# ericzzj1989/BALF

Hardware: NVIDIA B200
Metric: images/sec detect+NMS+top-k @640x480 (higher is better)
Workload: dtype fp16/tf32 operands (11-bit significand), fp32 accumulate

## Files before the change

### balf_b200/csrc/detector_tc.cuh

```cuda
#pragma once
#include <cuda_fp16.h>
#include "detector.cuh"
#include "umma.cuh"

namespace balf {
using namespace umma;

constexpr int kMerge32Ctas = 3;
constexpr int kRc16MinC = 32;
constexpr int TM = 128;
constexpr int NT2 = 256;
constexpr int kMaxSlot = 4;
constexpr int kMaxGemm = 6;

struct TcGemm {
    uint32_t goff;
    uint16_t nblk;
    uint16_t rows;
    uint16_t kb;
    uint16_t bias;
    uint16_t h16;
};
__host__ __device__ constexpr uint32_t tc_eb(int h16) { return h16 == 1 ? 2u : 4u; }
struct TcPlan {
// ... 180 lines not shown
            w_addr = r.wsm + slot * p.slot_bytes;
        }
        const uint64_t b_desc = desc_of(w_addr, b_lbo);
        fence_after_sync();
#pragma unroll
        for (int ks = 0; ks < KB / KSTEP; ++ks) {
            const uint32_t kchunk = (uint32_t)(b * KB) / EPC + (uint32_t)ks * 2u;
            const uint32_t a_off = ASW ? (kchunk / 8u) * (TM * 128u) + (kchunk % 8u) * 16u : kchunk * a_lbo;
            if (H16) mma_f16(d_tmem, a_desc + (a_off >> 4), b_desc + (((uint32_t)ks * 2u * b_lbo) >> 4), idesc, !(first && b == 0 && ks == 0));
            else mma_tf32(d_tmem, a_desc + (a_off >> 4), b_desc + (((uint32_t)ks * 2u * b_lbo) >> 4), idesc, !(first && b == 0 && ks == 0));
            if constexpr (X3) {
                mma_f16(d_tmem, a_desc + ((a_off + (uint32_t)(K / 8) * a_lbo) >> 4), b_desc + (((uint32_t)ks * 2u * b_lbo) >> 4), idesc, true);
                mma_f16(d_tmem, a_desc + (a_off >> 4), b_desc + ((((uint32_t)KB / 8u + (uint32_t)ks * 2u) * b_lbo) >> 4), idesc, true);
            }
        }
        if (BIAS && b + 1 == NBLK)
            mma_tf32(d_tmem, desc_of(ones_addr, TM * 16u), b_desc + ((((uint32_t)KB / EPC) * (X3 ? 2u : 1u) * b_lbo) >> 4), make_idesc_tf32(128, ROWS), true);
        if (!G::resident) { commit(&r.empty[slot]); ring_consumed<G::nslot>(r); }
    }
}

constexpr uint32_t kDescHiMn = ((uint32_t)(TM * 16u) >> 4) | (1u << 14);
__device__ __forceinline__ uint64_t desc_mn_of(uint32_t addr) {
    return ((uint64_t)kDescHiMn << 32) | (uint64_t)(((128u >> 4) << 16) | ((addr >> 4) & 0x3FFFu));
}
template <typename G, int GI, int C>
__device__ __forceinline__ void issue_mix_t(Ring& r, const TcPlan& p, uint32_t y_addr, uint32_t d_tmem) {
    uint32_t w_addr, slot = 0;
    if (G::resident) {
        w_addr = r.wsm + g_off<G>(GI);
    } else {
        ring_top_up<G::nslot>(r, p);
        slot = r.cslot;
        mbar_wait(&r.full[slot], r.cpar);
        w_addr = r.wsm + slot * p.slot_bytes;
    }
    fence_after_sync();
    constexpr uint32_t idesc = make_idesc_f16(64, C) | (1u << 16);
    constexpr uint32_t lo_off = (uint32_t)(C / 8) * TM * 16u;
    const uint64_t w_desc = desc_of(w_addr, 1024u);
    const uint64_t y_desc = desc_mn_of(y_addr);
#pragma unroll
    for (uint32_t u = 0; u < 2; ++u) {
#pragma unroll
        for (uint32_t ks = 0; ks < 4; ++ks) {
            const uint32_t yo = (32u * ks + 16u * u) * 16u;
            mma_f16(d_tmem + ((u * 16u) << 16), w_desc + ((ks * 2u * 1024u) >> 4), y_desc + (yo >> 4), idesc, ks > 0);
            if constexpr (G::x3) {
                mma_f16(d_tmem + ((u * 16u) << 16), w_desc + ((ks * 2u * 1024u) >> 4), y_desc + ((lo_off + yo) >> 4), idesc, true);
                mma_f16(d_tmem + ((u * 16u) << 16), w_desc + ((8192u + ks * 2u * 1024u) >> 4), y_desc + (yo >> 4), idesc, true);
            }
        }
    }
    if (!G::resident) { commit(&r.empty[slot]); ring_consumed<G::nslot>(r); }
}

__device__ __forceinline__ float ex2_approx(float x) {
    float y;
    asm("ex2.approx.ftz.f32 %0, %1;" : "=f"(y) : "f"(x));
    return y;
}
__device__ __forceinline__ unsigned long long pk2(float lo, float hi) {
    unsigned long long r;
    asm("mov.b64 %0, {%1, %2};" : "=l"(r) : "f"(lo), "f"(hi));
    return r;
}
__device__ __forceinline__ void upk2(unsigned long long r, float& lo, float& hi) { asm("mov.b64 {%0, %1}, %2;" : "=f"(lo), "=f"(hi) : "l"(r)); }
__device__ __forceinline__ unsigned long long fma2(unsigned long long a, unsigned long long b, unsigned long long c) {
    unsigned long long d;
    asm("fma.rn.f32x2 %0, %1, %2, %3;" : "=l"(d) : "l"(a), "l"(b), "l"(c));
    return d;
}
__device__ __forceinline__ unsigned long long add2(unsigned long long a, unsigned long long b) {
    unsigned long long d;
    asm("add.rn.f32x2 %0, %1, %2;" : "=l"(d) : "l"(a), "l"(b));
    return d;
}
__device__ __forceinline__ unsigned long long mul2(unsigned long long a, unsigned long long b) {
    unsigned long long d;
    asm("mul.rn.f32x2 %0, %1, %2;" : "=l"(d) : "l"(a), "l"(b));
    return d;
}
__device__ __forceinline__ void gelu_erf2(float& v0, float& v1) {
    const float t0 = fmaxf(-fabsf(v0), -5.6568542494923806f), t1 = fmaxf(-fabsf(v1), -5.6568542494923806f);
    const unsigned long long t = pk2(t0, t1);
    unsigned long long p = fma2(pk2(3.586947569e-04f, 3.586947569e-04f), t, pk2(6.316647399e-03f, 6.316647399e-03f));
    p = fma2(p, t, pk2(5.013782158e-02f, 5.013782158e-02f));
    p = fma2(p, t, pk2(-4.613807201e-01f, -4.613807201e-01f));
    p = fma2(p, t, pk2(1.150490999e+00f, 1.150490999e+00f));
    p = fma2(p, t, pk2(-1.0f, -1.0f));
    float p0, p1;
    upk2(p, p0, p1);
    const unsigned long long r = fma2(t, pk2(ex2_approx(p0), ex2_approx(p1)), pk2(fmaxf(v0, 0.0f), fmaxf(v1, 0.0f)));
    upk2(r, v0, v1);
}
template <int N, bool STATS>
__device__ __forceinline__ void gelu_row(float (&v)[N], float& sum, float& sq) {
    unsigned long long s2 = pk2(0.f, 0.f), q2 = pk2(0.f, 0.f);
#pragma unroll
    for (int i = 0; i < N; i += 2) {
        gelu_erf2(v[i], v[i + 1]);
        if (STATS) { const unsigned long long x = pk2(v[i], v[i + 1]); s2 = add2(s2, x); q2 = fma2(x, x, q2); }
    }
    if (STATS) { float a, b; upk2(s2, a, b); sum = a + b; upk2(q2, a, b); sq = a + b; }
}
template <int N>
__device__ __forceinline__ void norm_row(float (&v)[N], float rstd, float shift) {
    const unsigned long long r2 = pk2(rstd, rstd), h2 = pk2(shift, shift);
#pragma unroll
    for (int i = 0; i < N; i += 2) { const unsigned long long x = fma2(pk2(v[i], v[i + 1]), r2, h2); upk2(x, v[i], v[i + 1]); }
}
__device__ __forceinline__ float lrelu02(float v) { return v > 0.0f ? v : 0.2f * v; }

template <int CH>
__device__ __forceinline__ void ld_row(uint32_t taddr, float (&v)[CH]) {
    if constexpr (CH == 16) {
        tmem_ld16(taddr, v);
    } else {
#pragma unroll
        for (int c0 = 0; c0 < CH; c0 += 32) tmem_ld32(taddr + c0, *reinterpret_cast<float (*)[32]>(&v[c0]));
    }
    tmem_ld_wait();
}
template <int CH>
__device__ __forceinline__ void st_row(uint32_t taddr, const float (&v)[CH]) {
    if constexpr (CH == 16) {
        asm volatile(
            "tcgen05.st.sync.aligned.32x32b.x16.b32 [%0], {%1, %2, %3, %4, %5, %6, %7, %8, %9, %10, %11, %12, %13, %14, %15, %16};"
            :: "r"(taddr), "r"(__float_as_uint(v[0])), "r"(__float_as_uint(v[1])), "r"(__float_as_uint(v[2])), "r"(__float_as_uint(v[3])),
               "r"(__float_as_uint(v[4])), "r"(__float_as_uint(v[5])), "r"(__float_as_uint(v[6])), "r"(__float_as_uint(v[7])),
               "r"(__float_as_uint(v[8])), "r"(__float_as_uint(v[9])), "r"(__float_as_uint(v[10])), "r"(__float_as_uint(v[11])),
               "r"(__float_as_uint(v[12])), "r"(__float_as_uint(v[13])), "r"(__float_as_uint(v[14])), "r"(__float_as_uint(v[15]))
            : "memory");
    } else {
#pragma unroll
        for (int c0 = 0; c0 < CH; c0 += 32) tmem_st32(taddr + c0, *reinterpret_cast<const float (*)[32]>(&v[c0]));
    }
    tmem_st_wait();
}

template <int CH>
__device__ __forceinline__ void row_to_a(const float (&v)[CH], float* region, int row, int col0) {
#pragma unroll
    for (int j = 0; j < CH / 4; ++j)
        *reinterpret_cast<float4*>(region + ((size_t)(col0 / 4 + j) * TM + row) * 4) =
            to_tf32(make_float4(v[4 * j], v[4 * j + 1], v[4 * j + 2], v[4 * j + 3]));
}

__device__ __forceinline__ void split_h2(float a, float b, uint32_t& hi, uint32_t& lo) {
    asm("cvt.rn.satfinite.f16x2.f32 %0, %1, %2;" : "=r"(hi) : "f"(b), "f"(a));
    const float2 f = __half22float2(*reinterpret_cast<const __half2*>(&hi));
    asm("cvt.rn.satfinite.f16x2.f32 %0, %1, %2;" : "=r"(lo) : "f"(b - f.y), "f"(a - f.x));
}
template <int CH, int LOC = 0>
__device__ __forceinline__ void row_to_a16(const float (&v)[CH], float* region, int row, int col0) {
#pragma unroll
    for (int j = 0; j < CH / 8; ++j) {
        uint32_t h[4], l[4];
#pragma unroll
        for (int e = 0; e < 4; ++e) {
            if constexpr (LOC > 0) split_h2(v[8 * j + 2 * e], v[8 * j + 2 * e + 1], h[e], l[e]);
            else asm("cvt.rn.satfinite.f16x2.f32 %0, %1, %2;" : "=r"(h[e]) : "f"(v[8 * j + 2 * e + 1]), "f"(v[8 * j + 2 * e]));
        }
        *reinterpret_cast<uint4*>(region + ((size_t)(col0 / 8 + j) * TM + row) * 4) = make_uint4(h[0], h[1], h[2], h[3]);
        if constexpr (LOC > 0) *reinterpret_cast<uint4*>(region + ((size_t)(LOC + col0 / 8 + j) * TM + row) * 4) = make_uint4(l[0], l[1], l[2], l[3]);
    }
}
// ... 338 lines not shown
        }
        pf.v[0] = make_float4(v[0], v[1], v[2], v[3]);
    } else {
        constexpr int N = InputPf<CIN, TPR>::N;
        const float4* src = reinterpret_cast<const float4*>(xin + (img * npix + pix) * CIN) + half * N;
        if constexpr (PAIR) {
            pair_load<N>(src, valid, pf.v);
        } else {
#pragma unroll
            for (int j = 0; j < N; ++j) pf.v[j] = valid ? __ldg(src + j) : make_float4(0.f, 0.f, 0.f, 0.f);
        }
    }
}
template <int CIN, bool PAIR = true, int TPR = 2, int H16 = 0>
__device__ __forceinline__ void store_input_row(const InputPf<CIN, TPR>& pf, float* dst, int row, int half) {
    if constexpr (H16 == 3 && CIN >= 8) {
        constexpr int N16 = CIN / (8 * TPR);
#pragma unroll
        for (int j = 0; j < N16; ++j) *reinterpret_cast<float4*>(dst + ((size_t)(half * N16 + j) * TM + row) * 4) = pf.v[j];
        return;
    }
    if constexpr (CIN < 8) {
        if (half < 2) *reinterpret_cast<float4*>(dst + ((size_t)half * TM + row) * 4) = to_tf32(pf.v[0]);
    } else {
        constexpr int N = InputPf<CIN, TPR>::N;
#pragma unroll
        for (int j = 0; j < N; j += 2) {
            float4 c0 = pf.v[j], c1 = pf.v[j + 1];
            if constexpr (PAIR) pair_unswap(c0, c1);
            if constexpr (H16 != 0) {
                const float e[8] = {c0.x, c0.y, c0.z, c0.w, c1.x, c1.y, c1.z, c1.w};
                uint32_t h[4], l[4];
#pragma unroll
                for (int q = 0; q < 4; ++q) {
                    if constexpr (H16 == 2) split_h2(e[2 * q], e[2 * q + 1], h[q], l[q]);
                    else asm("cvt.rn.satfinite.f16x2.f32 %0, %1, %2;" : "=r"(h[q]) : "f"(e[2 * q + 1]), "f"(e[2 * q]));
                }
                *reinterpret_cast<uint4*>(dst + ((size_t)((half * N + j) / 2) * TM + row) * 4) = make_uint4(h[0], h[1], h[2], h[3]);
                if constexpr (H16 == 2)
                    *reinterpret_cast<uint4*>(dst + ((size_t)(CIN / 8 + (half * N + j) / 2) * TM + row) * 4) = make_uint4(l[0], l[1], l[2], l[3]);
            } else {
                *reinterpret_cast<float4*>(dst + ((size_t)(half * N + j) * TM + row) * 4) = to_tf32(c0);
                *reinterpret_cast<float4*>(dst + ((size_t)(half * N + j + 1) * TM + row) * 4) = to_tf32(c1);
            }
        }
    }
}


constexpr int kConv0Off = 64;
template <int CIN, int C>
__device__ __forceinline__ void conv0_stage_weights(const DownW& w, float* vec) {
    for (int i = threadIdx.x; i < CIN * C; i += NT2) vec[kConv0Off + i] = __ldg(w.conv0_w + i);
    for (int i = threadIdx.x; i < C; i += NT2) vec[kConv0Off + CIN * C + i] = __ldg(w.conv0_b + i);
}
template <int CIN, int C, int CH>
__device__ __forceinline__ void conv0_row(const float4 x, const float* vec, int col0, float (&v)[CH]) {
    const float xs[4] = {x.x, x.y, x.z, x.w};
    const float* cw = vec + kConv0Off + col0;
#pragma unroll
    for (int i = 0; i < CH; i += 4) {
        const float4 b = *reinterpret_cast<const float4*>(cw + CIN * C + i);
        unsigned long long a01 = pk2(b.x, b.y), a23 = pk2(b.z, b.w);
#pragma unroll
        for (int k = 0; k < CIN; ++k) {
            const float4 wv = *reinterpret_cast<const float4*>(cw + k * C + i);
            const unsigned long long xk = pk2(xs[k], xs[k]);
            a01 = fma2(pk2(wv.x, wv.y), xk, a01);
            a23 = fma2(pk2(wv.z, wv.w), xk, a23);
        }
        upk2(a01, v[i], v[i + 1]);
        upk2(a23, v[i + 2], v[i + 3]);
#pragma unroll
        for (int j = 0; j < 4; ++j) v[i + j] = fmaxf(v[i + j], 0.f);
    }
}

template <int C, int PX> struct BranchCfg {
    static constexpr int TPR = C == 32 ? 1 : C == 256 ? 4 : 2;
    static constexpr int groups = C == 32 ? 5 : C == 64 ? 2 : 1;
    static constexpr int NTG = TM * TPR;
    static constexpr int CH = C / TPR;
    static constexpr uint32_t region = (uint32_t)TM * C * (PX ? 4u : 2u);
    static constexpr bool park_u = C <= 128;
    static constexpr bool h16_out = C <= 128;
    static constexpr int col_u = 0;
    static constexpr int col_y = park_u ? C : 0;
    static constexpr int ncols = groups * tc_cols(col_y + 2 * C) > 512 ? col_y + 2 * C : tc_cols(col_y + 2 * C);
    static constexpr uint32_t xch = TPR == 1 ? 0u : 2u * TPR * TM * 8u;
    static constexpr int SC = TPR == 1 ? 16 : TPR == 4 ? (CH < 32 ? CH : 32) : (CH > 64 ? 64 : CH);
};

template <int CIN, int C, int BR, int PX>
__device__ __forceinline__ void tc_branch_body(const float* __restrict__ xin, const DownW& w, const TcPlan& plan, const UnitGeom& geo,
                                               float* __restrict__ out, float* __restrict__ scratch, unsigned char* smem) {
    using Cfg = BranchCfg<C, PX>;
    using G = BranchG<CIN, C, PX>;
    constexpr int CH = Cfg::CH, NG = Cfg::groups, TPR = Cfg::TPR, NTG = Cfg::NTG, SC = Cfg::SC;
    constexpr bool X3 = PX != 0;
    constexpr int LOC = X3 ? C / 8 : 0;
    constexpr bool XH = !X3 && CIN >= 8;
    constexpr bool CL16 = !Cfg::h16_out && !X3;
    float* const rt = CL16 ? scratch : out;
    constexpr int XM = XH ? 3 : X3 ? 2 : 1;
    static_assert(NG == 1 || G::resident, "tile groups share resident weights (no ring state per group)");
    static_assert(CH % SC == 0 && SC % 16 == 0, "sub-chunking");
    TcShared s = carve(smem, Cfg::region, plan, NG, Cfg::xch);
    const int grp = NG == 1 ? 0 : (int)(threadIdx.x / NTG);
    const int tid = threadIdx.x - grp * NTG, row = tid & (TM - 1), half = tid >> 7;
    const int vblock = (int)blockIdx.x * NG + grp, vgrid = (int)gridDim.x * NG;
    const int ntiles = (geo.total_units + 1) / 2;
    const uint32_t my_tiles = vblock < ntiles ? (ntiles - 1 - vblock) / vgrid + 1 : 0;
    const DownW::Branch& br = w.br[BR];
    if (grp == 0) {
        for (int i = tid; i < C; i += NTG) { s.vec[i] = __ldg(br.gn_w + i); s.vec[256 + i] = __ldg(br.gn_b + i); }
        for (int i = tid; i < 64; i += NTG) s.vec[512 + i] = __ldg(br.gd_b + i) + 1.0f;
        if constexpr (CIN < 8) {
            for (int i = tid; i < CIN * C; i += NTG) s.vec[kConv0Off + i] = __ldg(w.conv0_w + i);
            for (int i = tid; i < C; i += NTG) s.vec[kConv0Off + CIN * C + i] = __ldg(w.conv0_b + i);
        }
    }
    Ring ring;
    const bool w0 = __shfl_sync(0xffffffffu, tid >> 5, 0) == 0;
    tc_prologue<G::nslot>(s, tc_cols(Cfg::ncols * NG), ring, plan, my_tiles, w0 && grp == 0);
    if (NG > 1) {
        if (grp > 0 && w0 && elect_one()) mbar_wait(&s.full[0], 0);
        s.region += (size_t)grp * (Cfg::region / 4);
        s.xch += (size_t)grp * (Cfg::xch / 8);
        if (grp > 0) s.done = &s.gdone[grp];
    }
    const uint32_t tm = *s.tmem_slot + (uint32_t)(grp * Cfg::ncols);
    const uint32_t lane_base = tm + ((uint32_t)(row & ~31) << 16);
    const uint32_t region_addr = smem_u32(s.region), ones_addr = smem_u32(s.ones);
    const int ug = (row & 31) >> 4, tok = (row >> 5) * 16 + (row & 15);
    const int col0 = half * CH;
    const float* const mix_b1p = s.vec + 512 + tok;
    const int ostride = (BR == 0 ? geo.fw : 1) * C;
    const size_t npix = (size_t)geo.h * geo.w;
    uint32_t phase = 0, xb = 0;
    int it = 0;
    InputPf<CIN, TPR> pf;
    auto coords = [&](int tt, bool& vld, int& im, int& px) {
        const int un = 2 * tt + ug;
        vld = un < geo.total_units;
        im = vld ? fast_div(un, geo.upi, geo.inv_upi) : 0;
        px = unit_pixel<BR>(geo, vld ? un - im * geo.upi : 0, tok);
    };
    auto stats_of = [&](const float (&v)[CH], float& sum, float& sq) {
        unsigned long long s2 = pk2(0.f, 0.f), q2 = pk2(0.f, 0.f);
#pragma unroll
        for (int i = 0; i < CH; i += 2) {
            const unsigned long long x = pk2(v[i], v[i + 1]);
            s2 = add2(s2, x); q2 = fma2(x, x, q2);
        }
        float a, b;
        upk2(s2, a, b); sum = a + b;
        upk2(q2, a, b); sq = a + b;
    };
    bool nvld = false; int nim = 0, npx = 0;
    if (InputPf<CIN, TPR>::enabled && vblock < ntiles) {
        coords(vblock, nvld, nim, npx);
        fetch_input_row<CIN, true, TPR, XH>(xin, npix, (size_t)nim, npx, nvld, half, pf);
    }
    for (int t = vblock; t < ntiles; t += vgrid, ++it) {
        TC_TRACE(plan, it, 0);
        bool valid; int img, pix;
        if (InputPf<CIN, TPR>::enabled && (TPR > 1 || !X3)) { valid = nvld; img = nim; pix = npx; }
        else coords(t, valid, img, pix);
        float* orow = rt + ((size_t)img * npix + pix) * C + col0;
        float v[CH], rstd, shift;
        if constexpr (CIN < 8) {
            const float4 xv = pf.v[0];
            if (t + vgrid < ntiles) {
                coords(t + vgrid, nvld, nim, npx);
                fetch_input_row<CIN, true, TPR, XH>(xin, npix, (size_t)nim, npx, nvld, half, pf);
            }
            conv0_row<CIN, C, CH>(xv, s.vec, col0, v);
        } else {
            if (InputPf<CIN, TPR>::enabled) {
                store_input_row<CIN, true, TPR, XM>(pf, s.region, row, half);
                if (t + vgrid < ntiles) {
                    coords(t + vgrid, nvld, nim, npx);
                    fetch_input_row<CIN, true, TPR, XH>(xin, npix, (size_t)nim, npx, nvld, half, pf);
                }
            } else {
                load_input_row<CIN, TPR, XM>(xin, npix, (size_t)img, pix, valid, s.region, row, half);
            }
            TC_TRACE(plan, it, 1);
            sync_for_mma<NG, NTG>(grp);
            if (w0 && elect_one()) { issue_linear_t<G, BG_CONV0>(ring, plan, region_addr, ones_addr, tm + Cfg::col_y, true); commit(s.done); }
            TC_TRACE(plan, it, 2);
            wait_done_ring<G, NG, NTG>(s.done, phase, ring, plan, w0, grp);
            TC_TRACE(plan, it, 3);
            ld_row<CH>(lane_base + Cfg::col_y + col0, v);
#pragma unroll
            for (int i = 0; i < CH; ++i) v[i] = fmaxf(v[i], 0.f);
        }
        {
            float sum, sq;
            stats_of(v, sum, sq);
            row_stats<NG, TPR>(sum, sq, s.xch + (xb++ & 1) * TPR * TM, row, half, C, rstd, shift, grp);
            norm_row<CH>(v, rstd, shift);
            row_to_a16<CH, LOC>(v, s.region, row, col0);
        }
        TC_TRACE(plan, it, 4);
        sync_for_mma<NG, NTG>(grp);
        if (w0 && elect_one()) { issue_linear_t<G, BG_PD1>(ring, plan, region_addr, ones_addr, tm + Cfg::col_u, true); commit(s.done); }
        TC_TRACE(plan, it, 5);
        wait_done_ring<G, NG, NTG>(s.done, phase, ring, plan, w0, grp);
        TC_TRACE(plan, it, 6);
        {
            ld_row<CH>(lane_base + Cfg::col_u + col0, v);
            float sum = 0.f, sq = 0.f;
            gelu_row<CH, true>(v, sum, sq);
            if (Cfg::park_u) st_row<CH>(lane_base + Cfg::col_u + col0, v);
            else if constexpr (CH % 32 == 0 && !X3) oct_store<CH / 4>(rt, ((size_t)img * npix + pix) * C + col0, ostride, v, valid);
            else pair_store<CH / 4>(rt, ((size_t)img * npix + pix) * C + col0, v, valid);
            row_stats<NG, TPR>(sum, sq, s.xch + (xb++ & 1) * TPR * TM, row, half, C, rstd, shift, grp);
            norm_row<CH>(v, rstd, shift);
            row_to_a16<CH, LOC>(v, s.region, row, col0);
        }
        TC_TRACE(plan, it, 7);
        sync_for_mma<NG, NTG>(grp);
        if (w0 && elect_one()) {
            issue_linear_t<G, BG_D1A>(ring, plan, region_addr, ones_addr, tm + Cfg::col_y, true);
            issue_linear_t<G, BG_D1B>(ring, plan, region_addr, ones_addr, tm + Cfg::col_y + C, true);
            commit(s.done);
        }
        TC_TRACE(plan, it, 8);
        wait_done_ring<G, NG, NTG>(s.done, phase, ring, plan, w0, grp);
        TC_TRACE(plan, it, 9);
        {
            ld_row<CH>(lane_base + Cfg::col_y + col0, v);
            { float d0, d1; gelu_row<CH, false>(v, d0, d1); }
            st_row<CH>(lane_base + Cfg::col_y + col0, v);
            ld_row<CH>(lane_base + Cfg::col_y + C + col0, v);
            float sum = 0.f, sq = 0.f;
            gelu_row<CH, true>(v, sum, sq);
            row_stats<NG, TPR>(sum, sq, s.xch + (xb++ & 1) * TPR * TM, row, half, C, rstd, shift, grp);
            norm_row<CH>(v, rstd, shift);
#pragma unroll
            for (int i = 0; i < CH; i += 4) {
                const float4 gw = *reinterpret_cast<const float4*>(s.vec + col0 + i), gb = *reinterpret_cast<const float4*>(s.vec + 256 + col0 + i);
                upk2(fma2(pk2(v[i], v[i + 1]), pk2(gw.x, gw.y), pk2(gb.x, gb.y)), v[i], v[i + 1]);
                upk2(fma2(pk2(v[i + 2], v[i + 3]), pk2(gw.z, gw.w), pk2(gb.z, gb.w)), v[i + 2], v[i + 3]);
            }
            row_to_a16<CH, LOC>(v, s.region, row, col0);
        }
        TC_TRACE(plan, it, 10);
        sync_for_mma<NG, NTG>(grp);
        if (w0 && elect_one()) { issue_mix_t<G, BG_WM, C>(ring, plan, region_addr, tm + Cfg::col_y + C); commit(s.done); }
        TC_TRACE(plan, it, 11);
        wait_done_ring<G, NG, NTG>(s.done, phase, ring, plan, w0, grp);
        TC_TRACE(plan, it, 12);
        {
#pragma unroll 1
            for (int c = 0; c < CH; c += SC) {
                float y1[SC], y2[SC];
                ld_row<SC>(lane_base + Cfg::col_y + col0 + c, y1);
                ld_row<SC>(lane_base + Cfg::col_y + C + col0 + c, y2);
                const float mix_b1 = *mix_b1p;
                const unsigned long long b2 = pk2(mix_b1, mix_b1);
#pragma unroll
                for (int i = 0; i < SC; i += 2) upk2(mul2(pk2(y1[i], y1[i + 1]), add2(pk2(y2[i], y2[i + 1]), b2)), y2[i], y2[i + 1]);
                row_to_a16<SC, LOC>(y2, s.region, row, col0 + c);
            }
        }
        TC_TRACE(plan, it, 13);
        sync_for_mma<NG, NTG>(grp);
        if (w0 && elect_one()) { issue_linear_t<G, BG_D2>(ring, plan, region_addr, ones_addr, tm + Cfg::col_y, true); commit(s.done); }
        TC_TRACE(plan, it, 14);
        wait_done_ring<G, NG, NTG>(s.done, phase, ring, plan, w0, grp);
        TC_TRACE(plan, it, 15);
        {
            const bool odd = (threadIdx.x & 1) != 0;
            const size_t own_base = Cfg::h16_out ? ((size_t)img * npix + (pix & ~(TM - 1))) * C * (X3 ? 2 : 1)
                                                 : ((size_t)img * npix + pix) * C;
            const size_t oth_base = __shfl_xor_sync(0xffffffffu, (unsigned long long)own_base, 1);
            const size_t base_a = odd ? oth_base : own_base, base_b = odd ? own_base : oth_base;
            if constexpr (CL16 && CH % 64 == 0) {
                float hv[CH / 2];
#pragma unroll
                for (int c = 0; c < CH; c += SC) {
                    float a[SC];
                    ld_row<SC>(lane_base + Cfg::col_y + col0 + c, a);
#pragma unroll
                    for (int j0 = 0; j0 < SC / 4; j0 += 8) {
                        float4 t8[8];
                        pair_load<8>(reinterpret_cast<const float4*>(orow + c) + j0, valid, t8);
#pragma unroll
                        for (int j = 0; j < 8; j += 2) {
                            pair_unswap(t8[j], t8[j + 1]);
#pragma unroll
                            for (int u2 = 0; u2 < 2; ++u2) {
                                const float4 rr = t8[j + u2];
                                const int i = 4 * (j0 + j + u2);
                                uint32_t h0, h1;
                                asm("cvt.rn.satfinite.f16x2.f32 %0, %1, %2;" : "=r"(h0) : "f"(a[i + 1] + rr.y), "f"(a[i] + rr.x));
                                asm("cvt.rn.satfinite.f16x2.f32 %0, %1, %2;" : "=r"(h1) : "f"(a[i + 3] + rr.w), "f"(a[i + 2] + rr.z));
                                hv[(c + i) / 2] = __uint_as_float(h0);
                                hv[(c + i) / 2 + 1] = __uint_as_float(h1);
                            }
                        }
                    }
                }
                oct_store<CH / 8>(out, (((size_t)img * npix + pix) * C + col0) / 2, ostride / 2, hv, valid);
            } else
#pragma unroll 1
            for (int c = 0; c < CH; c += SC) {
                float a[SC], r[SC];
                ld_row<SC>(lane_base + Cfg::col_y + col0 + c, a);
                if (Cfg::park_u) ld_row<SC>(lane_base + Cfg::col_u + col0 + c, r);
                if constexpr (Cfg::h16_out) {
                    __half* tile = reinterpret_cast<__half*>(out) + own_base + (size_t)(pix & (TM - 1)) * 8;
#pragma unroll
                    for (int j = 0; j < SC / 8; ++j) {
                        uint32_t h[4], l[4];
#pragma unroll
                        for (int e = 0; e < 4; ++e) {
                            float lo, hi;
                            upk2(add2(pk2(a[8 * j + 2 * e], a[8 * j + 2 * e + 1]), pk2(r[8 * j + 2 * e], r[8 * j + 2 * e + 1])), lo, hi);
                            if constexpr (X3) split_h2(lo, hi, h[e], l[e]);
                            else asm("cvt.rn.satfinite.f16x2.f32 %0, %1, %2;" : "=r"(h[e]) : "f"(hi), "f"(lo));
                        }
                        if (valid) {
                            *reinterpret_cast<uint4*>(tile + (size_t)((col0 + c) / 8 + j) * (TM * 8)) = make_uint4(h[0], h[1], h[2], h[3]);
                            if constexpr (X3)
                                *reinterpret_cast<uint4*>(tile + (size_t)(C / 8 + (col0 + c) / 8 + j) * (TM * 8)) = make_uint4(l[0], l[1], l[2], l[3]);
                        }
                    }
                    continue;
                }
                float4 o[SC / 4];
                if constexpr (!Cfg::park_u) {
                    float4* rq = reinterpret_cast<float4*>(r);
#pragma unroll
                    for (int j0 = 0; j0 < SC / 4; j0 += 8) {
                        float4 t8[8];
                        pair_load<8>(reinterpret_cast<const float4*>(orow + c) + j0, valid, t8);
#pragma unroll
                        for (int j = 0; j < 8; j += 2) { pair_unswap(t8[j], t8[j + 1]); rq[j0 + j] = t8[j]; rq[j0 + j + 1] = t8[j + 1]; }
                    }
                }
#pragma unroll
                for (int j = 0; j < SC / 4; ++j) {
                    float4 res;
                    res = make_float4(r[4 * j], r[4 * j + 1], r[4 * j + 2], r[4 * j + 3]);
                    o[j] = make_float4(a[4 * j] + res.x, a[4 * j + 1] + res.y, a[4 * j + 2] + res.z, a[4 * j + 3] + res.w);
                    if (BR == 1 && !X3) o[j] = to_tf32_clean(o[j]);
                }
                if constexpr (SC % 32 == 0 && !X3) {
                    oct_store<SC / 4>(out, ((size_t)img * npix + pix) * C + col0 + c, ostride, reinterpret_cast<const float*>(o), valid);
                    continue;
                }
// ... 805 lines not shown
    if (g.bias)
        tc_pack_bias_kernel<<<cdiv(g.rows, 128), 128, 0, st>>>(wT, ld, n0, g.rows, k_real, bias, f.beta, f.alpha, f.add,
                                                               blob + g.goff + (size_t)g.rows * k_pad / (g.h16 == 1 ? 2 : 1));
    else if (p.ebias_off && bias) {
        const int slot = gi == MG_CONV0 ? 0 : gi == MG_PD2B ? 1 : gi == MG_RC1 ? 2 : 3;
        tc_pack_bias_kernel<<<cdiv(g.rows, 128), 128, 0, st>>>(wT, ld, n0, g.rows, k_real, bias, f.beta, f.alpha, f.add,
                                                               blob + p.ebias_off + (size_t)slot * g.rows * 4);
    }
}

int tc_pack_weights(const balf_detector_arch& a, const DetW& w, float* blob, cudaStream_t st) {
    BALF_CUDA_OK(cudaMemsetAsync(blob, 0, tc_blob_floats(a) * sizeof(float), st));
    const Fold none{nullptr, nullptr, nullptr, nullptr};
    for (int px = 0; px < 2; ++px) {
    TcPlans P;
    tc_build_plans(a, blob, &P, px);
    for (int l = 0; l < 4; ++l) {
        const int ci = a.dims[l], c = a.dims[l + 1];
        const DownW& d = w.down[l];
        for (int b = 0; b < 2; ++b) {
            const TcPlan& p = P.branch[l][b];
            const DownW::Branch& r = d.br[b];
            tc_pack_one(p, BG_CONV0, d.conv0_w, c, 0, ci, d.conv0_b, none, blob, st);
            tc_pack_one(p, BG_PD1, d.pd1_w, 2 * c, b * c, c, d.pd1_b, Fold{d.pn_w, d.pn_b, nullptr, nullptr}, blob, st);
            tc_pack_one(p, BG_D1A, r.d1_w, 2 * c, 0, c, r.d1_b, Fold{r.n_w, r.n_b, nullptr, nullptr}, blob, st);
            tc_pack_one(p, BG_D1B, r.d1_w, 2 * c, c, c, r.d1_b, Fold{r.n_w, r.n_b, nullptr, nullptr}, blob, st);
            tc_pack_one(p, BG_WM, r.gd_w, 64, 0, 64, nullptr, none, blob, st);
            tc_pack_one(p, BG_D2, r.d2_w, c, 0, c, r.d2_b, none, blob, st);
        }
        const TcPlan& m = P.merge[l];
        tc_pack_one(m, MG_CONV0, d.conv0_w, c, 0, ci, d.conv0_b, none, blob, st);
        tc_pack_one(m, MG_PD2A, d.pd2_w, c, 0, c, nullptr, none, blob, st);
        tc_pack_one(m, MG_PD2B, d.pd2_w + (size_t)c * c, c, 0, c, d.pd2_b, none, blob, st);
        tc_pack_one(m, MG_RC1, d.rc1_w, c, 0, c, d.rc1_b, Fold{d.rn_w, d.rn_b, nullptr, nullptr}, blob, st);
        tc_pack_one(m, MG_RC2, d.rc2_w, c, 0, c, d.rc2_b, none, blob, st);
    }
    tc_pack_one(P.head, HG_C2, w.down[3].c2_w, a.dims[4], 0, a.dims[4], w.down[3].c2_b, none, blob, st);
    tc_pack_one(P.head, HG_DENSE, w.head.w, kHeadPad, 0, a.dims[4], w.head.b, Fold{nullptr, nullptr, w.head.alpha, w.head.beta}, blob, st);
    }
    BALF_LAUNCH_OK();
    return 0;
}

#endif

static int g_num_sms = 0;
static int num_sms() {
    if (!g_num_sms) {
        int dev = 0;
        cudaGetDevice(&dev);
        cudaDeviceGetAttribute(&g_num_sms, cudaDevAttrMultiProcessorCount, dev);
        if (g_num_sms <= 0) g_num_sms = 148;
    }
    return g_num_sms;
}

template <typename K>
static int tc_launch_cfg(K kernel, size_t smem, int tmem_cols, int ntiles, int* grid, int groups = 1, int group_threads = NT2) {
    BALF_REQUIRE(smem <= 227 * 1024, "internal: tc kernel needs %zu bytes of shared memory", smem);
    BALF_CUDA_OK(cudaFuncSetAttribute(kernel, cudaFuncAttributeMaxDynamicSharedMemorySize, (int)smem));
    BALF_CUDA_OK(cudaFuncSetAttribute(kernel, cudaFuncAttributePreferredSharedMemoryCarveout, cudaSharedmemCarveoutMaxShared));
    cudaFuncAttributes fa;
    BALF_CUDA_OK(cudaFuncGetAttributes(&fa, kernel));
    const int regs_per_cta = ((fa.numRegs + 7) / 8 * 8) * group_threads * groups;
    ntiles = (ntiles + groups - 1) / groups;
    int per_sm = (int)((227 * 1024) / (smem + 1024));
    if (regs_per_cta > 0 && 65536 / regs_per_cta < per_sm) per_sm = 65536 / regs_per_cta;
    if (512 / tmem_cols < per_sm) per_sm = 512 / tmem_cols;
    if (per_sm < 1) per_sm = 1;
    const int cap = num_sms() * per_sm;
    *grid = ntiles < cap ? ntiles : cap;
    return 0;
}


template <int CIN, int C, int PX>
static int tc_launch_branches(const float* xin, const DownW& w, const TcPlans& P, int level, const UnitGeom& g, int ntiles,
                              float* u, float* v, float* su, float* sv, cudaStream_t st) {
    using Cfg = BranchCfg<C, PX>;
    constexpr int NG = Cfg::groups;
    int grid = 0;
    for (int b = 0; b < 2; ++b) {
        const TcPlan& p = P.branch[level][b];
        const size_t smem = tc_smem_bytes(Cfg::region, p, NG, Cfg::xch);
        if (b == 0) {
            if (int e = tc_launch_cfg(tc_branch_kernel<CIN, C, 0, PX>, smem, tc_cols(Cfg::ncols * NG), ntiles, &grid, NG, Cfg::NTG)) return e;
            ProfScope ps(C == 32 ? "det_branch_grid_c32" : C == 64 ? "det_branch_grid_c64" : C == 128 ? "det_branch_grid_c128" : "det_branch_grid_c256", st);
            tc_branch_kernel<CIN, C, 0, PX><<<grid, Cfg::NTG * NG, smem, st>>>(xin, w, p, g, u, su);
        } else {
            if (int e = tc_launch_cfg(tc_branch_kernel<CIN, C, 1, PX>, smem, tc_cols(Cfg::ncols * NG), ntiles, &grid, NG, Cfg::NTG)) return e;
            ProfScope ps(C == 32 ? "det_branch_block_c32" : C == 64 ? "det_branch_block_c64" : C == 128 ? "det_branch_block_c128" : "det_branch_block_c256", st);
            tc_branch_kernel<CIN, C, 1, PX><<<grid, Cfg::NTG * NG, smem, st>>>(xin, w, p, g, v, sv);
        }
    }
    return 0;
}

template <int CIN, int C, int PX>
static int tc_run_level(const float* xin, const DownW& w, const TcPlans& P, int level, int Bc, int h, int wd,
                        float* u, float* v, float* r, float* q, float* partial, cudaStream_t st, int r16) {
    UnitGeom g{h, wd, h / 8, wd / 8, h * wd / 64, Bc * (h * wd / 64), 1.0f / (float)(h * wd / 64), 1.0f / (float)(wd / 8), 1.0f / (float)(wd / 8)};
    BALF_REQUIRE(g.total_units < (1 << 23), "internal: %d units in one pass exceed the fast_div range", g.total_units);
    const int ntiles = (g.total_units + 1) / 2;
    int grid = 0;
    BALF_REQUIRE((plan_matches<BranchG<CIN, C, PX>>(P.branch[level][0]) && plan_matches<BranchG<CIN, C, PX>>(P.branch[level][1]) &&
                  plan_matches<MergeG<CIN, C, PX>>(P.merge[level])), "internal: compile-time and packed GEMM plans differ (level %d)", level);
    if (int e = tc_launch_branches<CIN, C, PX>(xin, w, P, level, g, ntiles, u, v, r, q, st)) return e;
    if constexpr (C <= 64) {
        const TcPlan& p = P.merge[level];
        BALF_REQUIRE(g.total_units % 2 == 0, "internal: odd unit count at stage %d", level);
        const size_t smem = tc_smem_bytes(MergeBulkCfg<CIN, C, PX>::region, p, 1, MergeBulkCfg<CIN, C, PX>::xch);
        if (int e = tc_launch_cfg(tc_merge_bulk_kernel<CIN, C, PX>, smem, MergeBulkCfg<CIN, C, PX>::ncols, ntiles, &grid)) return e;
        ProfScope ps(C == 32 ? "det_merge_c32" : "det_merge_c64", st);
        tc_merge_bulk_kernel<CIN, C, PX><<<grid, NT2, smem, st>>>(xin, w, p, g, u, v, r, q, partial);
    } else {
        const TcPlan& p = P.merge[level];
        BALF_REQUIRE((!MergeCfg<C, PX>::bulk_uv || g.total_units % 2 == 0), "internal: odd unit count at stage %d", level);
        const size_t smem = tc_smem_bytes(MergeCfg<C, PX>::region, p, 1, MergeCfg<C, PX>::xch);
        if (int e = tc_launch_cfg(tc_merge_kernel<CIN, C, PX>, smem, MergeCfg<C, PX>::ncols, ntiles, &grid, 1, MergeCfg<C, PX>::NT)) return e;
        ProfScope ps(C == 128 ? "det_merge_c128" : "det_merge_c256", st);
        tc_merge_kernel<CIN, C, PX><<<grid, MergeCfg<C, PX>::NT, smem, st>>>(xin, p, g, u, v, r, q, partial, r16);
    }
    BALF_COUNT_LAUNCH(3);
    BALF_LAUNCH_OK();
    return 0;
}

template <int PX>
int tc_level_px(int level, const float* xin, const DownW& w, const balf_detector_arch& a, const float* blob,
                int Bc, int h, int wd, float* u, float* v, float* r, float* q, float* partial, cudaStream_t st, int r16) {
    TcPlans P;
    tc_build_plans(a, blob, &P, PX);
    switch (level) {
        case 0: return tc_run_level<3, 32, PX>(xin, w, P, 0, Bc, h, wd, u, v, r, q, partial, st, r16);
        case 1: return tc_run_level<32, 64, PX>(xin, w, P, 1, Bc, h, wd, u, v, r, q, partial, st, r16);
        case 2: return tc_run_level<64, 128, PX>(xin, w, P, 2, Bc, h, wd, u, v, r, q, partial, st, r16);
        default: return tc_run_level<128, 256, PX>(xin, w, P, 3, Bc, h, wd, u, v, r, q, partial, st, r16);
    }
}
template <int PX>
int tc_head_px(const float* r, const float* q, const float* scale, const balf_detector_arch& a,
               const float* blob, int Bc, int hc, int wc, float* logits, float* prob, cudaStream_t st, int r16) {
    TcPlans P;
    tc_build_plans(a, blob, &P, PX);
    UnitGeom g{hc, wc, hc / 8, wc / 8, hc * wc / 64, Bc * (hc * wc / 64), 1.0f / (float)(hc * wc / 64), 1.0f / (float)(wc / 8), 1.0f / (float)(wc / 8)};
    BALF_REQUIRE(g.total_units < (1 << 23), "internal: %d units in one pass exceed the fast_div range", g.total_units);
    const int ntiles = (g.total_units + 1) / 2;
    const size_t smem = tc_smem_bytes((uint32_t)TM * 256 * 4, P.head);
    int grid = 0;
    BALF_REQUIRE((plan_matches<HeadG<256, PX>>(P.head)), "internal: compile-time and packed GEMM plans differ (head)");
    if (int e = tc_launch_cfg(tc_head_kernel<256, PX>, smem, 512, ntiles, &grid)) return e;
    {
        ProfScope ps("det_head", st);
        tc_head_kernel<256, PX><<<grid, NT2, smem, st>>>(r, q, scale, P.head, g, a.cell, logits, prob, PX ? 0 : r16);
    }
    BALF_COUNT_LAUNCH(1);
    BALF_LAUNCH_OK();
    return 0;
}

#ifdef BALF_TC_MAIN
extern template int tc_level_px<1>(int, const float*, const DownW&, const balf_detector_arch&, const float*, int, int, int, float*, float*,
                                   float*, float*, float*, cudaStream_t, int);
extern template int tc_head_px<1>(const float*, const float*, const float*, const balf_detector_arch&, const float*, int, int, int, float*,
                                  float*, cudaStream_t, int);

int tc_run_level_dispatch(int level, const float* xin, const DownW& w, const balf_detector_arch& a, const float* blob,
// ... 21 lines not shown
```

Baseline: 5238.

## Double-buffer C32 operand region and overlap next tile's conv0 with MMAs

For the C=32 branch (where conv.0 runs on CUDA cores), the shared operand region is doubled so the next tile's conv0, row-norm and fp16 staging run while the final linear MMA of the current tile is in flight. The GELU pass over the first TMEM half moves after the mix MMA issue so it overlaps that MMA. The erf clamp in gelu_erf2 is removed to save an instruction per pair. Costs are more shared memory per CTA, which can reduce occupancy, and possible range issues in the polynomial for large |x| without the clamp.

Result: faster. 5388, median of 6 (+2.9%).

```diff
diff --git a/balf_b200/csrc/detector_tc.cuh b/balf_b200/csrc/detector_tc.cuh
--- a/balf_b200/csrc/detector_tc.cuh
+++ b/balf_b200/csrc/detector_tc.cuh
@@ -286,7 +286,7 @@
     return d;
 }
 __device__ __forceinline__ void gelu_erf2(float& v0, float& v1) {
-    const float t0 = fmaxf(-fabsf(v0), -5.6568542494923806f), t1 = fmaxf(-fabsf(v1), -5.6568542494923806f);
+    const float t0 = -fabsf(v0), t1 = -fabsf(v1);
     const unsigned long long t = pk2(t0, t1);
     unsigned long long p = fma2(pk2(3.586947569e-04f, 3.586947569e-04f), t, pk2(6.316647399e-03f, 6.316647399e-03f));
     p = fma2(p, t, pk2(5.013782158e-02f, 5.013782158e-02f));
@@ -791,6 +791,7 @@
     static constexpr int NTG = TM * TPR;
     static constexpr int CH = C / TPR;
     static constexpr uint32_t region = (uint32_t)TM * C * (PX ? 4u : 2u);
+    static constexpr int nbuf = C == 32 ? 2 : 1;
     static constexpr bool park_u = C <= 128;
     static constexpr bool h16_out = C <= 128;
     static constexpr int col_u = 0;
@@ -814,7 +815,8 @@
     constexpr int XM = XH ? 3 : X3 ? 2 : 1;
     static_assert(NG == 1 || G::resident, "tile groups share resident weights (no ring state per group)");
     static_assert(CH % SC == 0 && SC % 16 == 0, "sub-chunking");
-    TcShared s = carve(smem, Cfg::region, plan, NG, Cfg::xch);
+    static_assert((Cfg::nbuf == 2) == (CIN < 8), "two operand regions exactly where conv.0 runs on the CUDA cores");
+    TcShared s = carve(smem, Cfg::nbuf * Cfg::region, plan, NG, Cfg::xch);
     const int grp = NG == 1 ? 0 : (int)(threadIdx.x / NTG);
     const int tid = threadIdx.x - grp * NTG, row = tid & (TM - 1), half = tid >> 7;
     const int vblock = (int)blockIdx.x * NG + grp, vgrid = (int)gridDim.x * NG;
@@ -834,13 +836,13 @@
     tc_prologue<G::nslot>(s, tc_cols(Cfg::ncols * NG), ring, plan, my_tiles, w0 && grp == 0);
     if (NG > 1) {
         if (grp > 0 && w0 && elect_one()) mbar_wait(&s.full[0], 0);
-        s.region += (size_t)grp * (Cfg::region / 4);
+        s.region += (size_t)grp * (Cfg::nbuf * Cfg::region / 4);
         s.xch += (size_t)grp * (Cfg::xch / 8);
         if (grp > 0) s.done = &s.gdone[grp];
     }
     const uint32_t tm = *s.tmem_slot + (uint32_t)(grp * Cfg::ncols);
     const uint32_t lane_base = tm + ((uint32_t)(row & ~31) << 16);
-    const uint32_t region_addr = smem_u32(s.region), ones_addr = smem_u32(s.ones);
+    const uint32_t region0_addr = smem_u32(s.region), ones_addr = smem_u32(s.ones);
     const int ug = (row & 31) >> 4, tok = (row >> 5) * 16 + (row & 15);
     const int col0 = half * CH;
     const float* const mix_b1p = s.vec + 512 + tok;
@@ -871,29 +873,49 @@
         coords(vblock, nvld, nim, npx);
         fetch_input_row<CIN, true, TPR, XH>(xin, npix, (size_t)nim, npx, nvld, half, pf);
     }
+    bool cvld = false; int cim = 0, cpx = 0;
+    auto stage1_input = [&](int tn, float* dst) {
+        if constexpr (CIN < 8) {
+            const float4 xv = pf.v[0];
+            cvld = nvld; cim = nim; cpx = npx;
+            if (tn + vgrid < ntiles) {
+                coords(tn + vgrid, nvld, nim, npx);
+                fetch_input_row<CIN, true, TPR, XH>(xin, npix, (size_t)nim, npx, nvld, half, pf);
+            }
+            float v[CH], rstd, shift, sum, sq;
+            conv0_row<CIN, C, CH>(xv, s.vec, col0, v);
+            stats_of(v, sum, sq);
+            row_stats<NG, TPR>(sum, sq, s.xch + (xb++ & 1) * TPR * TM, row, half, C, rstd, shift, grp);
+            norm_row<CH>(v, rstd, shift);
+            row_to_a16<CH, LOC>(v, dst, row, col0);
+        }
+    };
+    if constexpr (CIN < 8) {
+        if (vblock < ntiles) stage1_input(vblock, s.region);
+    }
     for (int t = vblock; t < ntiles; t += vgrid, ++it) {
         TC_TRACE(plan, it, 0);
+        const uint32_t rb = (uint32_t)(it & (Cfg::nbuf - 1));
+        float* const region = s.region + (size_t)rb * (Cfg::region / 4);
+        const uint32_t region_addr = region0_addr + rb * Cfg::region;
         bool valid; int img, pix;
-        if (InputPf<CIN, TPR>::enabled && (TPR > 1 || !X3)) { valid = nvld; img = nim; pix = npx; }
-        else coords(t, valid, img, pix);
+        if (InputPf<CIN, TPR>::enabled && (TPR > 1 || !X3)) {
+            if constexpr (CIN < 8) { valid = cvld; img = cim; pix = cpx; }
+            else { valid = nvld; img = nim; pix = npx; }
+        } else {
+            coords(t, valid, img, pix);
+        }
         float* orow = rt + ((size_t)img * npix + pix) * C + col0;
         float v[CH], rstd, shift;
-        if constexpr (CIN < 8) {
-            const float4 xv = pf.v[0];
-            if (t + vgrid < ntiles) {
-                coords(t + vgrid, nvld, nim, npx);
-                fetch_input_row<CIN, true, TPR, XH>(xin, npix, (size_t)nim, npx, nvld, half, pf);
-            }
-            conv0_row<CIN, C, CH>(xv, s.vec, col0, v);
-        } else {
+        if constexpr (CIN >= 8) {
             if (InputPf<CIN, TPR>::enabled) {
-                store_input_row<CIN, true, TPR, XM>(pf, s.region, row, half);
+                store_input_row<CIN, true, TPR, XM>(pf, region, row, half);
                 if (t + vgrid < ntiles) {
                     coords(t + vgrid, nvld, nim, npx);
                     fetch_input_row<CIN, true, TPR, XH>(xin, npix, (size_t)nim, npx, nvld, half, pf);
                 }
             } else {
-                load_input_row<CIN, TPR, XM>(xin, npix, (size_t)img, pix, valid, s.region, row, half);
+                load_input_row<CIN, TPR, XM>(xin, npix, (size_t)img, pix, valid, region, row, half);
             }
             TC_TRACE(plan, it, 1);
             sync_for_mma<NG, NTG>(grp);
@@ -904,13 +926,11 @@
             ld_row<CH>(lane_base + Cfg::col_y + col0, v);
 #pragma unroll
             for (int i = 0; i < CH; ++i) v[i] = fmaxf(v[i], 0.f);
-        }
-        {
             float sum, sq;
             stats_of(v, sum, sq);
             row_stats<NG, TPR>(sum, sq, s.xch + (xb++ & 1) * TPR * TM, row, half, C, rstd, shift, grp);
             norm_row<CH>(v, rstd, shift);
-            row_to_a16<CH, LOC>(v, s.region, row, col0);
+            row_to_a16<CH, LOC>(v, region, row, col0);
         }
         TC_TRACE(plan, it, 4);
         sync_for_mma<NG, NTG>(grp);
@@ -927,7 +947,7 @@
             else pair_store<CH / 4>(rt, ((size_t)img * npix + pix) * C + col0, v, valid);
             row_stats<NG, TPR>(sum, sq, s.xch + (xb++ & 1) * TPR * TM, row, half, C, rstd, shift, grp);
             norm_row<CH>(v, rstd, shift);
-            row_to_a16<CH, LOC>(v, s.region, row, col0);
+            row_to_a16<CH, LOC>(v, region, row, col0);
         }
         TC_TRACE(plan, it, 7);
         sync_for_mma<NG, NTG>(grp);
@@ -940,9 +960,6 @@
         wait_done_ring<G, NG, NTG>(s.done, phase, ring, plan, w0, grp);
         TC_TRACE(plan, it, 9);
         {
-            ld_row<CH>(lane_base + Cfg::col_y + col0, v);
-            { float d0, d1; gelu_row<CH, false>(v, d0, d1); }
-            st_row<CH>(lane_base + Cfg::col_y + col0, v);
             ld_row<CH>(lane_base + Cfg::col_y + C + col0, v);
             float sum = 0.f, sq = 0.f;
             gelu_row<CH, true>(v, sum, sq);
@@ -954,12 +971,17 @@
                 upk2(fma2(pk2(v[i], v[i + 1]), pk2(gw.x, gw.y), pk2(gb.x, gb.y)), v[i], v[i + 1]);
                 upk2(fma2(pk2(v[i + 2], v[i + 3]), pk2(gw.z, gw.w), pk2(gb.z, gb.w)), v[i + 2], v[i + 3]);
             }
-            row_to_a16<CH, LOC>(v, s.region, row, col0);
+            row_to_a16<CH, LOC>(v, region, row, col0);
         }
         TC_TRACE(plan, it, 10);
         sync_for_mma<NG, NTG>(grp);
         if (w0 && elect_one()) { issue_mix_t<G, BG_WM, C>(ring, plan, region_addr, tm + Cfg::col_y + C); commit(s.done); }
         TC_TRACE(plan, it, 11);
+        {
+            ld_row<CH>(lane_base + Cfg::col_y + col0, v);
+            { float d0, d1; gelu_row<CH, false>(v, d0, d1); }
+            st_row<CH>(lane_base + Cfg::col_y + col0, v);
+        }
         wait_done_ring<G, NG, NTG>(s.done, phase, ring, plan, w0, grp);
         TC_TRACE(plan, it, 12);
         {
@@ -972,13 +994,16 @@
                 const unsigned long long b2 = pk2(mix_b1, mix_b1);
 #pragma unroll
                 for (int i = 0; i < SC; i += 2) upk2(mul2(pk2(y1[i], y1[i + 1]), add2(pk2(y2[i], y2[i + 1]), b2)), y2[i], y2[i + 1]);
-                row_to_a16<SC, LOC>(y2, s.region, row, col0 + c);
+                row_to_a16<SC, LOC>(y2, region, row, col0 + c);
             }
         }
         TC_TRACE(plan, it, 13);
         sync_for_mma<NG, NTG>(grp);
         if (w0 && elect_one()) { issue_linear_t<G, BG_D2>(ring, plan, region_addr, ones_addr, tm + Cfg::col_y, true); commit(s.done); }
         TC_TRACE(plan, it, 14);
+        if constexpr (CIN < 8) {
+            if (t + vgrid < ntiles) stage1_input(t + vgrid, s.region + (size_t)((it + 1) & 1) * (Cfg::region / 4));
+        }
         wait_done_ring<G, NG, NTG>(s.done, phase, ring, plan, w0, grp);
         TC_TRACE(plan, it, 15);
         {
@@ -1950,7 +1975,7 @@
     int grid = 0;
     for (int b = 0; b < 2; ++b) {
         const TcPlan& p = P.branch[level][b];
-        const size_t smem = tc_smem_bytes(Cfg::region, p, NG, Cfg::xch);
+        const size_t smem = tc_smem_bytes(Cfg::nbuf * Cfg::region, p, NG, Cfg::xch);
         if (b == 0) {
             if (int e = tc_launch_cfg(tc_branch_kernel<CIN, C, 0, PX>, smem, tc_cols(Cfg::ncols * NG), ntiles, &grid, NG, Cfg::NTG)) return e;
             ProfScope ps(C == 32 ? "det_branch_grid_c32" : C == 64 ? "det_branch_grid_c64" : C == 128 ? "det_branch_grid_c128" : "det_branch_grid_c256", st);
```
